# manyeyes/K2TransducerAsr

Measured on AMD Instinct MI355X. Metric: RTFx (audio-sec/wall-sec) offline Zipformer greedy, higher is better.
Workload: dtype f32

## Files before the change

### k2transducerasr_amd/csrc/attn.hip

```cpp
#include "kernels.h"

namespace k2hip {

typedef float f32x16 __attribute__((ext_vector_type(16)));

namespace {

constexpr int PH = 4;
constexpr int R = 32;

template <int NG>
__global__ __launch_bounds__(512, 4) void k_attn_scores_softmax(const float* __restrict__ qkp, int ld,
                                                             const float* __restrict__ pp, float* __restrict__ aw, int B,
                                                             int T, int Tp, int H, int lds_stride, int koff0, int poff0) {
    constexpr int QH = 8 * NG;
    extern __shared__ __attribute__((aligned(16))) float S[];
    const int tid = threadIdx.x, lane = tid & 63, wave = tid >> 6;
    const int li = lane & 31, lh = lane >> 5;
    const int i0 = blockIdx.x * R, b = blockIdx.y, h = blockIdx.z;
    const float* base = qkp + (long long)b * T * ld;
    const int qoff = h * QH, koff = koff0 + h * QH, poff = poff0 + h * PH;
    const int ppld = H * PH;

    float4 fq[NG];
// ... 111 lines not shown
                if (k >= nk) break;
                v[rr][k].x = __expf(v[rr][k].x - mx); v[rr][k].y = __expf(v[rr][k].y - mx);
                v[rr][k].z = __expf(v[rr][k].z - mx); v[rr][k].w = __expf(v[rr][k].w - mx);
                sum += (v[rr][k].x + v[rr][k].y) + (v[rr][k].z + v[rr][k].w);
            }
#pragma unroll
            for (int o = 32; o > 0; o >>= 1) sum += __shfl_xor(sum, o);
            const float inv = 1.0f / sum;
            float* orow = out + (long long)i * Tp;
#pragma unroll
            for (int k = 0; k < 4; k++) {
                const int j4 = lane * 4 + 256 * k;
                if (k < nk && j4 < Tp) *reinterpret_cast<float4*>(orow + j4) = make_float4(v[rr][k].x * inv, v[rr][k].y * inv, v[rr][k].z * inv, v[rr][k].w * inv);
            }
        }
        return;
    }
    for (int rr = 0; rr < 4; rr++) {
        int rl = wave * 4 + rr, i = i0 + rl;
        if (i >= T) break;
        float* srow = S + rl * lds_stride;
        float mx = -INFINITY;
        for (int j = lane; j < T; j += 64) mx = fmaxf(mx, srow[j]);
        mx = wave_max_dpp(mx);
        float sum = 0.f;
        for (int j = lane; j < T; j += 64) {
            float e = __expf(srow[j] - mx);
            srow[j] = e;
            sum += e;
        }
#pragma unroll
        for (int o = 32; o > 0; o >>= 1) sum += __shfl_xor(sum, o);
        float inv = 1.0f / sum;
        float* orow = out + (long long)i * Tp;
        for (int j4 = lane * 4; j4 < Tp; j4 += 256) {
            float4 v;
            v.x = (j4 + 0 < T) ? srow[j4 + 0] * inv : 0.f;
            v.y = (j4 + 1 < T) ? srow[j4 + 1] * inv : 0.f;
            v.z = (j4 + 2 < T) ? srow[j4 + 2] * inv : 0.f;
            v.w = (j4 + 3 < T) ? srow[j4 + 3] * inv : 0.f;
            *reinterpret_cast<float4*>(orow + j4) = v;
        }
    }
}

template <int NG>
__global__ __launch_bounds__(256) void k_attn_scores_softmax_long(const float* __restrict__ qkp, int ld, const float* __restrict__ pp,
                                                                  float* __restrict__ aw, int B, int T, int Tp, int H, int koff0, int poff0) {
    constexpr int QH = 8 * NG;
    __shared__ float smx[4][R], ssm[4][R];
    const int tid = threadIdx.x, lane = tid & 63, wave = tid >> 6;
    const int li = lane & 31, lh = lane >> 5;
    const int i0 = blockIdx.x * R, b = blockIdx.y, h = blockIdx.z;
    const float* base = qkp + (long long)b * T * ld;
    const int qoff = h * QH, koff = koff0 + h * QH, poff = poff0 + h * PH;
    const int ppld = H * PH;
    float4 fq[NG];
    {
        int row = i0 + li;
#pragma unroll
        for (int g = 0; g < NG; g++) {
            fq[g] = make_float4(0.f, 0.f, 0.f, 0.f);
            if (row < T) fq[g] = *reinterpret_cast<const float4*>(base + (long long)row * ld + qoff + 8 * g + 4 * lh);
        }
    }
    float4 pr[16];
#pragma unroll
    for (int r = 0; r < 16; r++) {
        int row = i0 + (r & 3) + 8 * (r >> 2) + 4 * lh;
        pr[r] = make_float4(0.f, 0.f, 0.f, 0.f);
        if (row < T) pr[r] = *reinterpret_cast<const float4*>(base + (long long)row * ld + poff);
    }
    const int njt = (T + 31) / 32;
    float rm[16], rs[16];
#pragma unroll
    for (int r = 0; r < 16; r++) { rm[r] = -INFINITY; rs[r] = 0.f; }
    float* out = aw + (((long long)h * B + b) * T) * Tp;
    for (int pass = 0; pass < 2; pass++) {
        for (int jt = wave; jt < njt; jt += 4) {
            const int j = jt * 32 + li;
            float4 fk[NG];
#pragma unroll
            for (int g = 0; g < NG; g++) {
                fk[g] = make_float4(0.f, 0.f, 0.f, 0.f);
                if (j < T) fk[g] = *reinterpret_cast<const float4*>(base + (long long)j * ld + koff + 8 * g + 4 * lh);
            }
            f32x16 acc;
#pragma unroll
            for (int r = 0; r < 16; r++) acc[r] = 0.f;
#pragma unroll
            for (int g = 0; g < NG; g++) {
                acc = __builtin_amdgcn_mfma_f32_32x32x2f32(fq[g].x, fk[g].x, acc, 0, 0, 0);
                acc = __builtin_amdgcn_mfma_f32_32x32x2f32(fq[g].y, fk[g].y, acc, 0, 0, 0);
                acc = __builtin_amdgcn_mfma_f32_32x32x2f32(fq[g].z, fk[g].z, acc, 0, 0, 0);
                acc = __builtin_amdgcn_mfma_f32_32x32x2f32(fq[g].w, fk[g].w, acc, 0, 0, 0);
            }
            if (j < T) {
#pragma unroll
                for (int r = 0; r < 16; r++) {
                    const int i = i0 + (r & 3) + 8 * (r >> 2) + 4 * lh;
                    if (i >= T) continue;
                    const float4 e = *reinterpret_cast<const float4*>(pp + (long long)(T - 1 - i + j) * ppld + h * PH);
                    const float sc = acc[r] + pr[r].x * e.x + pr[r].y * e.y + pr[r].z * e.z + pr[r].w * e.w;
                    if (pass == 0) {
                        const float m = fmaxf(rm[r], sc);
                        rs[r] = rs[r] * __expf(rm[r] - m) + __expf(sc - m);
                        rm[r] = m;
                    } else {
                        out[(long long)i * Tp + j] = __expf(sc - rm[r]) * rs[r];
                    }
                }
            }
        }
        if (pass == 0) {
#pragma unroll
            for (int r = 0; r < 16; r++) {
                float m = rm[r], sv = rs[r];
#pragma unroll
                for (int o = 16; o > 0; o >>= 1) {
                    const float om = __shfl_xor(m, o), os = __shfl_xor(sv, o);
                    const float nm = fmaxf(m, om);
                    sv = (m == -INFINITY ? 0.f : sv * __expf(m - nm)) + (om == -INFINITY ? 0.f : os * __expf(om - nm));
                    m = nm;
                }
                if (li == 0) {
                    const int rl = (r & 3) + 8 * (r >> 2) + 4 * lh;
                    smx[wave][rl] = m;
                    ssm[wave][rl] = sv;
                }
            }
            __syncthreads();
#pragma unroll
            for (int r = 0; r < 16; r++) {
                const int rl = (r & 3) + 8 * (r >> 2) + 4 * lh;
                float m = -INFINITY;
                for (int w = 0; w < 4; w++) m = fmaxf(m, smx[w][rl]);
                float sv = 0.f;
                for (int w = 0; w < 4; w++)
                    if (smx[w][rl] != -INFINITY) sv += ssm[w][rl] * __expf(smx[w][rl] - m);
                rm[r] = m;
                rs[r] = 1.0f / sv;
            }
        }
    }
    for (int idx = tid; idx < R * (Tp - T); idx += 256) {
        const int rl = idx / (Tp - T), c = T + idx % (Tp - T);
        if (i0 + rl < T) out[(long long)(i0 + rl) * Tp + c] = 0.f;
    }
}


typedef float f32x4 __attribute__((ext_vector_type(4)));

template <bool RING, bool PROJ = false>
__global__ __launch_bounds__(256) void k_attn_av_out(const float* __restrict__ aw, const float* __restrict__ v,
                                                     const float* __restrict__ wout, const float* __restrict__ bias,
                                                     float* __restrict__ x, int B, int T, int KL, int Tp, int Tk, int H, int vh,
                                                     int D, int tiles_per_z, RingRef ring, const float* __restrict__ newrows,
                                                     const float* __restrict__ xin = nullptr, const float* __restrict__ win = nullptr,
                                                     const float* __restrict__ bin = nullptr) {
    extern __shared__ float avs[];
    const int HV = H * vh, AS = HV + 1;
    const int tid = threadIdx.x, lane = tid & 63, wave = tid >> 6;
    const int b = blockIdx.y, i0 = blockIdx.x * 16;
    const int n = lane & 15, kq = lane >> 4;
    const float* xres = PROJ ? xin : x;
    if (RING) {
        float* rb = ring.pool + (long long)ring.slots[b] * ring.slot_stride + ring.off;
        const int head = (int)(((long long)ring.chunks[b] * T) % KL), h4 = HV >> 2;
        if (PROJ) {
            float* xs = avs + 16 * AS + ((4 - ((16 * AS) & 3)) & 3);
            const int XS = D + 4, d4 = D >> 2;
            for (int e = tid; e < 16 * d4; e += 256) {
                const int r = e / d4, c = (e % d4) * 4;
                *reinterpret_cast<float4*>(xs + r * XS + c) =
                    r < T ? *reinterpret_cast<const float4*>(xin + ((long long)b * T + r) * D + c) : make_float4(0.f, 0.f, 0.f, 0.f);
            }
            __syncthreads();
            const float* xr = xs + n * XS + 4 * kq;
            for (int ct = wave; 16 * ct < HV; ct += 4) {
                const int col = 16 * ct + n;
                const float* wr = win + (long long)min(col, HV - 1) * D + 4 * kq;
                f32x4 acc0 = {0.f, 0.f, 0.f, 0.f}, acc1 = {0.f, 0.f, 0.f, 0.f};
                for (int k0 = 0; k0 < D; k0 += 64) {
                    float4 w4[4], a4[4];
                    const int ns = min(4, (D - k0) >> 4);
#pragma unroll
                    for (int q = 0; q < 4; q++) w4[q] = q < ns ? *reinterpret_cast<const float4*>(wr + k0 + 16 * q) : make_float4(0.f, 0.f, 0.f, 0.f);
#pragma unroll
                    for (int q = 0; q < 4; q++) a4[q] = q < ns ? *reinterpret_cast<const float4*>(xr + k0 + 16 * q) : make_float4(0.f, 0.f, 0.f, 0.f);
#pragma unroll
                    for (int q = 0; q < 4; q += 2) {
                        acc0 = __builtin_amdgcn_mfma_f32_16x16x4f32(a4[q].x, w4[q].x, acc0, 0, 0, 0);
                        acc1 = __builtin_amdgcn_mfma_f32_16x16x4f32(a4[q + 1].x, w4[q + 1].x, acc1, 0, 0, 0);
                        acc0 = __builtin_amdgcn_mfma_f32_16x16x4f32(a4[q].y, w4[q].y, acc0, 0, 0, 0);
                        acc1 = __builtin_amdgcn_mfma_f32_16x16x4f32(a4[q + 1].y, w4[q + 1].y, acc1, 0, 0, 0);
                        acc0 = __builtin_amdgcn_mfma_f32_16x16x4f32(a4[q].z, w4[q].z, acc0, 0, 0, 0);
                        acc1 = __builtin_amdgcn_mfma_f32_16x16x4f32(a4[q + 1].z, w4[q + 1].z, acc1, 0, 0, 0);
                        acc0 = __builtin_amdgcn_mfma_f32_16x16x4f32(a4[q].w, w4[q].w, acc0, 0, 0, 0);
                        acc1 = __builtin_amdgcn_mfma_f32_16x16x4f32(a4[q + 1].w, w4[q + 1].w, acc1, 0, 0, 0);
                    }
                }
                if (col < HV) {
                    const float bc = bin[col];
#pragma unroll
                    for (int e = 0; e < 4; e++) {
                        const int r = 4 * kq + e;
                        if (r < T) rb[(long long)((head + r) % KL) * HV + col] = (acc0[e] + acc1[e]) + bc;
                    }
                }
            }
        } else {
            for (int e = tid; e < T * h4; e += 256) {
                const int r = e / h4, c = (e % h4) * 4;
                *reinterpret_cast<float4*>(rb + (long long)((head + r) % KL) * HV + c) =
                    *reinterpret_cast<const float4*>(newrows + ((long long)b * T + r) * HV + c);
            }
        }
        __syncthreads();
        v = rb;
    } else {
        v += (long long)b * KL * HV;
    }
    const int row_a = min(i0 + n, T - 1);
    const bool ncol = n < vh;
    for (int h = wave; h < H; h += 4) {
        const float* arow = aw + (((long long)h * B + b) * T + row_a) * Tp + 4 * kq;
        const float* vb = v + (long long)(4 * kq) * HV + h * vh + (ncol ? n : 0);
        f32x4 acc0 = {0.f, 0.f, 0.f, 0.f}, acc1 = {0.f, 0.f, 0.f, 0.f};
        float4 a4[4], a4n[4];
        float bv[4][4], bvn[4][4];
        auto load_step = [&](float4* ad, float (*bd)[4], int k0) {
#pragma unroll
            for (int g = 0; g < 4; g++) {
                const int kb = k0 + 16 * g + 4 * kq;
                ad[g] = kb < Tp ? *reinterpret_cast<const float4*>(arow + k0 + 16 * g) : make_float4(0.f, 0.f, 0.f, 0.f);
#pragma unroll
                for (int m = 0; m < 4; m++) bd[g][m] = (ncol && kb + m < KL) ? vb[(long long)(k0 + 16 * g + m) * HV] : 0.f;
            }
        };
        load_step(a4, bv, 0);
        for (int k0 = 0; k0 < Tk; k0 += 64) {
            if (k0 + 64 < Tk) load_step(a4n, bvn, k0 + 64);
#pragma unroll
            for (int g = 0; g < 4; g++) {
                if (g & 1) {
                    acc1 = __builtin_amdgcn_mfma_f32_16x16x4f32(a4[g].x, bv[g][0], acc1, 0, 0, 0);
                    acc1 = __builtin_amdgcn_mfma_f32_16x16x4f32(a4[g].y, bv[g][1], acc1, 0, 0, 0);
                    acc1 = __builtin_amdgcn_mfma_f32_16x16x4f32(a4[g].z, bv[g][2], acc1, 0, 0, 0);
                    acc1 = __builtin_amdgcn_mfma_f32_16x16x4f32(a4[g].w, bv[g][3], acc1, 0, 0, 0);
                } else {
                    acc0 = __builtin_amdgcn_mfma_f32_16x16x4f32(a4[g].x, bv[g][0], acc0, 0, 0, 0);
                    acc0 = __builtin_amdgcn_mfma_f32_16x16x4f32(a4[g].y, bv[g][1], acc0, 0, 0, 0);
                    acc0 = __builtin_amdgcn_mfma_f32_16x16x4f32(a4[g].z, bv[g][2], acc0, 0, 0, 0);
                    acc0 = __builtin_amdgcn_mfma_f32_16x16x4f32(a4[g].w, bv[g][3], acc0, 0, 0, 0);
                }
            }
#pragma unroll
            for (int g = 0; g < 4; g++) {
                a4[g] = a4n[g];
#pragma unroll
                for (int m = 0; m < 4; m++) bv[g][m] = bvn[g][m];
            }
        }
        if (ncol) {
#pragma unroll
            for (int e = 0; e < 4; e++) avs[(4 * kq + e) * AS + h * vh + n] = acc0[e] + acc1[e];
        }
    }
    __syncthreads();
    constexpr int MAXC = 8;
    const int nch = (HV + 15) >> 4;
    float4 av4[MAXC];
#pragma unroll
    for (int c = 0; c < MAXC; c++) {
        const int kb = 16 * c + 4 * kq;
        const float* ar = avs + n * AS + kb;
        av4[c] = (c < nch && kb < HV) ? make_float4(ar[0], ar[1], ar[2], ar[3]) : make_float4(0.f, 0.f, 0.f, 0.f);
    }
    const int ct0 = blockIdx.z * tiles_per_z, ct1 = min(D >> 4, ct0 + tiles_per_z);
    float4 wc[MAXC], wn[MAXC];
    auto load_w = [&](float4* dst, int ct) {
        const float* wr = wout + (long long)(ct * 16 + n) * HV + 4 * kq;
#pragma unroll
        for (int c = 0; c < MAXC; c++)
            dst[c] = (c < nch && 16 * c + 4 * kq < HV) ? *reinterpret_cast<const float4*>(wr + 16 * c) : make_float4(0.f, 0.f, 0.f, 0.f);
    };
    float xa[4], xb[4], ba = 0.f, bb = 0.f;
    auto load_x = [&](float* dst, float& bdst, int ct) {
        const int col = ct * 16 + n;
        bdst = bias[col];
#pragma unroll
        for (int e = 0; e < 4; e++) {
            const int i = i0 + 4 * kq + e;
            dst[e] = i < T ? xres[((long long)b * T + i) * D + col] : 0.f;
        }
    };
    auto tile = [&](const float4* w, const float* xr, float bv, int ct) {
        const int col = ct * 16 + n;
        f32x4 acc0 = {0.f, 0.f, 0.f, 0.f}, acc1 = {0.f, 0.f, 0.f, 0.f};
#pragma unroll
        for (int c = 0; c < MAXC; c++) {
            if (c < nch) {
                if (c & 1) {
                    acc1 = __builtin_amdgcn_mfma_f32_16x16x4f32(av4[c].x, w[c].x, acc1, 0, 0, 0);
                    acc1 = __builtin_amdgcn_mfma_f32_16x16x4f32(av4[c].y, w[c].y, acc1, 0, 0, 0);
                    acc1 = __builtin_amdgcn_mfma_f32_16x16x4f32(av4[c].z, w[c].z, acc1, 0, 0, 0);
                    acc1 = __builtin_amdgcn_mfma_f32_16x16x4f32(av4[c].w, w[c].w, acc1, 0, 0, 0);
                } else {
                    acc0 = __builtin_amdgcn_mfma_f32_16x16x4f32(av4[c].x, w[c].x, acc0, 0, 0, 0);
                    acc0 = __builtin_amdgcn_mfma_f32_16x16x4f32(av4[c].y, w[c].y, acc0, 0, 0, 0);
                    acc0 = __builtin_amdgcn_mfma_f32_16x16x4f32(av4[c].z, w[c].z, acc0, 0, 0, 0);
                    acc0 = __builtin_amdgcn_mfma_f32_16x16x4f32(av4[c].w, w[c].w, acc0, 0, 0, 0);
                }
            }
        }
        float o[4];
#pragma unroll
        for (int e = 0; e < 4; e++) o[e] = acc0[e] + acc1[e] + bv + xr[e];
        asm volatile("" : "+v"(o[0]), "+v"(o[1]), "+v"(o[2]), "+v"(o[3]));
        float* xp = x + ((long long)b * T + i0 + 4 * kq) * D + col;
#pragma unroll
        for (int e = 0; e < 4; e++)
            if (i0 + 4 * kq + e < T) xp[(long long)e * D] = o[e];
    };
    int ct = ct0 + wave;
    if (ct < ct1) {
        load_w(wc, ct);
        load_x(xa, ba, ct);
    }
    while (ct < ct1) {
        if (ct + 4 < ct1) {
            load_w(wn, ct + 4);
            load_x(xb, bb, ct + 4);
        }
        tile(wc, xa, ba, ct);
        ct += 4;
        if (ct >= ct1) break;
        if (ct + 4 < ct1) {
            load_w(wc, ct + 4);
            load_x(xa, ba, ct + 4);
        }
        tile(wn, xb, bb, ct);
        ct += 4;
    }
}


template <int NS, int NT, bool MULTI = false>
__global__ __launch_bounds__(NT) void k_nonlin_av_out(const float* __restrict__ aw, const float* __restrict__ hid, int ldh,
                                                      const float* __restrict__ wout, const float* __restrict__ bias,
                                                      float* __restrict__ x, int B, int T, int KL, int Tp, int Hc, int D,
                                                      int tiles_per_z, RingRef ring) {
    extern __shared__ float cs_[];
    constexpr int NWV = NT / 64;
    const int CS = ((Hc + 15) & ~15) + 4;
    const int tid = threadIdx.x, lane = tid & 63, wave = tid >> 6;
    const int b = blockIdx.y;
    const int n = lane & 15, kq = lane >> 4;
    float* rb = ring.pool + (long long)ring.slots[b] * ring.slot_stride + ring.off;
    {
        const int head = (int)(((long long)ring.chunks[b] * T) % KL), h4 = Hc >> 2;
        for (int e = tid; e < T * h4; e += NT) {
            const int r = e / h4, c = (e % h4) * 4;
            const float* p = hid + ((long long)b * T + r) * ldh + c;
            const float4 sg = *reinterpret_cast<const float4*>(p), v = *reinterpret_cast<const float4*>(p + Hc);
            *reinterpret_cast<float4*>(rb + (long long)((head + r) % KL) * Hc + c) =
                make_float4(v.x * tanhf(sg.x), v.y * tanhf(sg.y), v.z * tanhf(sg.z), v.w * tanhf(sg.w));
        }
    }
    __syncthreads();
    const int row_a = min(n, T - 1);
    const float* arow = aw + ((long long)b * T + row_a) * Tp + 4 * kq;
    for (int ct = wave; ct * 16 < Hc; ct += NWV) {
        const bool cok = ct * 16 + n < Hc;
        const float* vb = rb + (long long)(4 * kq) * Hc + (cok ? ct * 16 + n : 0);
        f32x4 acc0 = {0.f, 0.f, 0.f, 0.f}, acc1 = {0.f, 0.f, 0.f, 0.f};
        const int trips = MULTI ? (KL + 64 * NS - 1) / (64 * NS) : 1;
        for (int tr = 0; tr < trips; tr++) {
        const int k0 = 64 * NS * tr;
        float4 a4[NS][4];
        float bv[NS][4][4];
#pragma unroll
        for (int s = 0; s < NS; s++)
#pragma unroll
            for (int g = 0; g < 4; g++) {
                const int kb = k0 + 64 * s + 16 * g + 4 * kq;
                a4[s][g] = kb < Tp ? *reinterpret_cast<const float4*>(arow + k0 + 64 * s + 16 * g) : make_float4(0.f, 0.f, 0.f, 0.f);
#pragma unroll
                for (int m = 0; m < 4; m++) bv[s][g][m] = (cok && kb + m < KL) ? vb[(long long)(k0 + 64 * s + 16 * g + m) * Hc] : 0.f;
            }
#pragma unroll
        for (int s = 0; s < NS; s++)
#pragma unroll
            for (int g = 0; g < 4; g++) {
                if (g & 1) {
                    acc1 = __builtin_amdgcn_mfma_f32_16x16x4f32(a4[s][g].x, bv[s][g][0], acc1, 0, 0, 0);
                    acc1 = __builtin_amdgcn_mfma_f32_16x16x4f32(a4[s][g].y, bv[s][g][1], acc1, 0, 0, 0);
                    acc1 = __builtin_amdgcn_mfma_f32_16x16x4f32(a4[s][g].z, bv[s][g][2], acc1, 0, 0, 0);
                    acc1 = __builtin_amdgcn_mfma_f32_16x16x4f32(a4[s][g].w, bv[s][g][3], acc1, 0, 0, 0);
                } else {
                    acc0 = __builtin_amdgcn_mfma_f32_16x16x4f32(a4[s][g].x, bv[s][g][0], acc0, 0, 0, 0);
                    acc0 = __builtin_amdgcn_mfma_f32_16x16x4f32(a4[s][g].y, bv[s][g][1], acc0, 0, 0, 0);
                    acc0 = __builtin_amdgcn_mfma_f32_16x16x4f32(a4[s][g].z, bv[s][g][2], acc0, 0, 0, 0);
                    acc0 = __builtin_amdgcn_mfma_f32_16x16x4f32(a4[s][g].w, bv[s][g][3], acc0, 0, 0, 0);
                }
            }
        }
#pragma unroll
        for (int e = 0; e < 4; e++) {
            const int r = 4 * kq + e;
            const float gate = (cok && r < T) ? hid[((long long)b * T + r) * ldh + 2 * Hc + ct * 16 + n] : 0.f;
            cs_[r * CS + ct * 16 + n] = (acc0[e] + acc1[e]) * gate;
        }
    }
    __syncthreads();
    if (!wout) {
        const int h4 = Hc >> 2;
        for (int e = tid; e < T * h4; e += NT) {
            const int r = e / h4, c = (e % h4) * 4;
            *reinterpret_cast<float4*>(x + ((long long)b * T + r) * Hc + c) = *reinterpret_cast<const float4*>(cs_ + r * CS + c);
        }
        return;
    }
    const int ct0 = blockIdx.z * tiles_per_z, ct1 = min(D >> 4, ct0 + tiles_per_z);
    const float* ar = cs_ + n * CS + 4 * kq;
    for (int ct = ct0 + wave; ct < ct1; ct += NWV) {
        const int col = ct * 16 + n;
        const float* wr = wout + (long long)col * Hc + 4 * kq;
        const float bvv = bias[col];
        float xr[4];
#pragma unroll
        for (int e = 0; e < 4; e++) {
            const int i = 4 * kq + e;
            xr[e] = i < T ? x[((long long)b * T + i) * D + col] : 0.f;
        }
        f32x4 acc0 = {0.f, 0.f, 0.f, 0.f}, acc1 = {0.f, 0.f, 0.f, 0.f};
        for (int c0 = 0; c0 < Hc; c0 += 64) {
            float4 w4[4], a4[4];
#pragma unroll
            for (int g = 0; g < 4; g++) {
                const bool ok = c0 + 16 * g + 4 * kq < Hc;
                w4[g] = ok ? *reinterpret_cast<const float4*>(wr + c0 + 16 * g) : make_float4(0.f, 0.f, 0.f, 0.f);
                a4[g] = ok ? *reinterpret_cast<const float4*>(ar + c0 + 16 * g) : make_float4(0.f, 0.f, 0.f, 0.f);
            }
#pragma unroll
            for (int g = 0; g < 4; g++) {
                if (g & 1) {
                    acc1 = __builtin_amdgcn_mfma_f32_16x16x4f32(a4[g].x, w4[g].x, acc1, 0, 0, 0);
                    acc1 = __builtin_amdgcn_mfma_f32_16x16x4f32(a4[g].y, w4[g].y, acc1, 0, 0, 0);
                    acc1 = __builtin_amdgcn_mfma_f32_16x16x4f32(a4[g].z, w4[g].z, acc1, 0, 0, 0);
                    acc1 = __builtin_amdgcn_mfma_f32_16x16x4f32(a4[g].w, w4[g].w, acc1, 0, 0, 0);
                } else {
                    acc0 = __builtin_amdgcn_mfma_f32_16x16x4f32(a4[g].x, w4[g].x, acc0, 0, 0, 0);
                    acc0 = __builtin_amdgcn_mfma_f32_16x16x4f32(a4[g].y, w4[g].y, acc0, 0, 0, 0);
                    acc0 = __builtin_amdgcn_mfma_f32_16x16x4f32(a4[g].z, w4[g].z, acc0, 0, 0, 0);
                    acc0 = __builtin_amdgcn_mfma_f32_16x16x4f32(a4[g].w, w4[g].w, acc0, 0, 0, 0);
                }
            }
        }
        float o[4];
#pragma unroll
        for (int e = 0; e < 4; e++) o[e] = acc0[e] + acc1[e] + bvv + xr[e];
        float* xp = x + ((long long)b * T + 4 * kq) * D + col;
#pragma unroll
        for (int e = 0; e < 4; e++)
            if (4 * kq + e < T) xp[(long long)e * D] = o[e];
    }
}

}

template <int NG>
static void attn_scores_launch(const Ctx& ctx, const float* qkp, int ld, const float* pp, float* aw, int B, int T, int Tp, int H, int koff0,
                               int poff0) {
    int lds_stride = Tp + 4;
    size_t lds = sizeof(float) * R * lds_stride;
    const bool force_long = tunables().attn_long != 0;
    if (lds > 160 * 1024 || force_long) {
        hipLaunchKernelGGL(k_attn_scores_softmax_long<NG>, dim3(cdiv(T, R), B, H), dim3(256), 0, ctx.stream, qkp, ld, pp, aw, B, T, Tp, H, koff0,
                           poff0);
        K2_HIP(hipGetLastError());
        return;
    }
    static LdsAttrOnce lds_attr;
    lds_attr.ensure(k_attn_scores_softmax<NG>, 160 * 1024);
    dim3 grid(cdiv(T, R), B, H);
    hipLaunchKernelGGL(k_attn_scores_softmax<NG>, grid, dim3(512), lds, ctx.stream, qkp, ld, pp, aw, B, T, Tp, H, lds_stride, koff0, poff0);
    K2_HIP(hipGetLastError());
}

void attn_scores_softmax(const Ctx& ctx, const float* qkp, int ld, const float* pp, float* aw, int B, int T, int Tp, int H, int qh, int koff0,
                         int poff0) {
    K2_REQUIRE(Tp % 4 == 0 && Tp >= T, "attn: Tp=%d must be T=%d rounded up to 4", Tp, T);
    if (koff0 < 0) koff0 = H * qh;
    if (poff0 < 0) poff0 = 2 * H * qh;
    K2_REQUIRE(koff0 % 4 == 0 && poff0 % 4 == 0 && ld % 4 == 0, "attn: operand offsets must be multiples of 4 floats");
    ctx.add_flops(0.0, 2.0 * (qh + PH) * (double)T * T * B * H, 0);
    if (ctx.dry) return;
    switch (qh) {
        case 32: attn_scores_launch<4>(ctx, qkp, ld, pp, aw, B, T, Tp, H, koff0, poff0); break;
        case 24: attn_scores_launch<3>(ctx, qkp, ld, pp, aw, B, T, Tp, H, koff0, poff0); break;
        case 16: attn_scores_launch<2>(ctx, qkp, ld, pp, aw, B, T, Tp, H, koff0, poff0); break;
        default: failf(K2HIP_ERR_UNSUPPORTED, "attention head size %d unsupported (16, 24, 32)", qh);
    }
}

bool attn_av_out(const Ctx& ctx, const float* aw, const float* v, const float* wout, const float* bias, float* x, int B, int T, int KL, int Tp,
                 int H, int vh, int D) {
    const int HV = H * vh, Tk = (KL + 63) & ~63;
    const bool off = tunables().no_fused_av != 0;
    if (off || vh > 16 || HV % 4 != 0 || HV > 128 || D % 16 != 0 || Tp % 4 != 0 || Tp < KL) return false;
    ctx.add_flops(0.0, 2.0 * B * (double)T * HV * (KL + D), 0);
    if (ctx.dry) return true;
    const int strips = cdiv(T, 16) * B, ntile = D / 16;
    int cs = std::max(1, std::min(4, 512 / std::max(1, strips)));
    cs = std::min(cs, ntile);
    const int tiles_per_z = cdiv(ntile, cs);
    cs = cdiv(ntile, tiles_per_z);
    const size_t lds = sizeof(float) * 16 * (HV + 1);
    hipLaunchKernelGGL(k_attn_av_out<false>, dim3(cdiv(T, 16), B, cs), dim3(256), lds, ctx.stream, aw, v, wout, bias, x, B, T, KL, Tp, Tk, H, vh,
                       D, tiles_per_z, RingRef(), nullptr);
    K2_HIP(hipGetLastError());
    return true;
}

bool attn_av_out_ring(const Ctx& ctx, const float* aw, const RingRef& vals, const float* newrows, const float* wout, const float* bias, float* x,
                      int B, int T, int KL, int Tp, int H, int vh, int D) {
    const int HV = H * vh, Tk = (KL + 63) & ~63;
    K2_REQUIRE(vh <= 16 && HV % 4 == 0 && HV <= 128 && D % 16 == 0 && Tp % 4 == 0 && Tp >= KL && T <= 16,
               "attn_av_out_ring: shape H=%d vh=%d D=%d T=%d KL=%d unsupported", H, vh, D, T, KL);
    ctx.add_flops(0.0, 2.0 * B * (double)T * HV * (KL + D), 0);
    if (ctx.dry) return true;
    const int strips = B, ntile = D / 16;
    int cs = std::max(1, std::min(4, 512 / std::max(1, strips)));
    cs = std::min(cs, ntile);
    const int tiles_per_z = cdiv(ntile, cs);
    cs = cdiv(ntile, tiles_per_z);
    const size_t lds = sizeof(float) * 16 * (HV + 1);
    hipLaunchKernelGGL(k_attn_av_out<true>, dim3(1, B, cs), dim3(256), lds, ctx.stream, aw, nullptr, wout, bias, x, B, T, KL, Tp, Tk, H, vh, D,
                       tiles_per_z, vals, newrows);
    K2_HIP(hipGetLastError());
    return true;
}

void attn_proj_av_out_ring(const Ctx& ctx, const float* aw, const RingRef& vals, const float* xin, const float* win, const float* bin,
                           const float* wout, const float* bias, float* xout, int B, int T, int KL, int Tp, int H, int vh, int D) {
    const int HV = H * vh, Tk = (KL + 63) & ~63;
    K2_REQUIRE(vh <= 16 && HV % 4 == 0 && HV <= 128 && D % 32 == 0 && Tp % 4 == 0 && Tp >= KL && T <= 16,
               "attn_proj_av_out_ring: shape H=%d vh=%d D=%d T=%d KL=%d unsupported", H, vh, D, T, KL);
    K2_REQUIRE(ctx.dry || xin != xout, "attn_proj_av_out_ring: input and output must be different buffers");
    ctx.add_flops(0.0, 2.0 * B * (double)T * HV * (KL + D) + 2.0 * B * (double)T * HV * D, 0);
    if (ctx.dry) return;
    const int strips = B, ntile = D / 16;
    int cs = std::max(1, std::min(4, 512 / std::max(1, strips)));
    cs = std::min(cs, ntile);
    const int tiles_per_z = cdiv(ntile, cs);
    cs = cdiv(ntile, tiles_per_z);
    const size_t lds = sizeof(float) * (16 * (HV + 1) + 4 + 16 * (D + 4));
    K2_REQUIRE(lds <= 64 * 1024, "attn_proj_av_out_ring: D=%d too wide", D);
    hipLaunchKernelGGL((k_attn_av_out<true, true>), dim3(1, B, cs), dim3(256), lds, ctx.stream, aw, nullptr, wout, bias, xout, B, T, KL, Tp, Tk, H, vh,
                       D, tiles_per_z, vals, nullptr, xin, win, bin);
    K2_HIP(hipGetLastError());
}

void nonlin_av_out_ring(const Ctx& ctx, const float* aw, const RingRef& cache, const float* hid, int ldh, const float* wout, const float* bias,
                        float* x, int B, int T, int KL, int Tp, int Hc, int D) {
    K2_REQUIRE(Hc % 4 == 0 && D % 16 == 0 && Tp % 4 == 0 && Tp >= KL && T <= 16 && ldh % 4 == 0 && ldh >= 3 * Hc,
               "nonlin_av_out_ring: shape Hc=%d D=%d T=%d KL=%d unsupported", Hc, D, T, KL);
    ctx.add_flops(0.0, 2.0 * B * (double)T * Hc * (KL + D), 0);
    const size_t lds = sizeof(float) * 16 * (((Hc + 15) & ~15) + 4);
    K2_REQUIRE(lds <= 64 * 1024, "nonlin_av_out_ring: Hc=%d too wide", Hc);
    const int ns = (KL + 63) / 64;
    K2_REQUIRE(ns >= 1, "nonlin_av_out_ring: no keys");
    if (ctx.dry) return;
    const int ntile = D / 16;
    int cs = std::max(1, std::min(4, 512 / std::max(1, B)));
    cs = std::min(cs, ntile);
    if (!wout) cs = 1;
    const int tiles_per_z = cdiv(ntile, cs);
    cs = cdiv(ntile, tiles_per_z);
    const bool wide = (Hc + 15) / 16 > 8;
#define K2_NONLIN_LAUNCH(NS_, NT_)                                                                                                   \
    hipLaunchKernelGGL((k_nonlin_av_out<NS_, NT_>), dim3(1, B, cs), dim3(NT_), lds, ctx.stream, aw, hid, ldh, wout, bias, x, B, T, KL, Tp, Hc, \
                       D, tiles_per_z, cache)
    switch (ns) {
        case 1: if (wide) K2_NONLIN_LAUNCH(1, 1024); else K2_NONLIN_LAUNCH(1, 512); break;
        case 2: if (wide) K2_NONLIN_LAUNCH(2, 1024); else K2_NONLIN_LAUNCH(2, 512); break;
        case 3: if (wide) K2_NONLIN_LAUNCH(3, 1024); else K2_NONLIN_LAUNCH(3, 512); break;
        case 4: K2_NONLIN_LAUNCH(4, 512); break;
        default:
            hipLaunchKernelGGL((k_nonlin_av_out<4, 512, true>), dim3(1, B, cs), dim3(512), lds, ctx.stream, aw, hid, ldh, wout, bias, x, B, T, KL,
                               Tp, Hc, D, tiles_per_z, cache);
            break;
    }
#undef K2_NONLIN_LAUNCH
    K2_HIP(hipGetLastError());
}

}
```

### k2transducerasr_amd/csrc/kernels.h

```cpp
#pragma once
#include "ctc_prefix_layout.h"
#include "common.h"

namespace k2hip {

#ifdef K2HIP_DEV
#define K2HIP_DEV_SWITCH(name, def) int name = def
#else
#define K2HIP_DEV_SWITCH(name, def) static constexpr int name = def
#endif
struct Tunables {
    int no_glu_epilogue = 0;
    int attn_long = 0;
    int no_fused_av = 0;
    int fused_vproj_min_t = 4;
    int no_fused_vproj = 0;
    int no_fused_conv = 0;
    int conformer_gemm_scores = 0;
    int dw7_tiled = 0;
    int dw1d_tt = 0;
    int lstm_seq = 0;
    int greedy_one_part = 0;
    int greedy_parts = 0;
    int beam_launches = 0;
    int beam_parts = 0;
    int beam_hyp_global = 0;
    int beam_trace = 0;
    int search_rounds = -1;
    int test_greedy_timeout = 0;
    int decoder_table_mb = 1024;
    int screen_min_v = 1024;
    int screen_count = 0;
    int max_streams = 0;
    K2HIP_DEV_SWITCH(gemm_cfg, -1);
    K2HIP_DEV_SWITCH(xcd_panels, 0);
    K2HIP_DEV_SWITCH(greedy_stamps, 0);
    K2HIP_DEV_SWITCH(conformer_stamps, 0);
};
void tunables_init_from_env();
const Tunables& tunables();
bool tunables_set(const char* env_name, int value);

struct GemmStats {
    double flops = 0;
    double total_flops = 0;
    int launches = 0;
    float ms = 0;
};

struct GemmLaunchRec {
    int M, N, K, batch, act, res, kind;
    float us;
};

struct GreedyLaunch;
struct Ctx {
    std::vector<GemmLaunchRec>* gemm_log = nullptr;
    GreedyLaunch* greedy_rec = nullptr;
    hipStream_t stream = nullptr;
    Arena* arena = nullptr;
    bool dry = false;
    bool one_part = false;
    bool instrument = false;
    GemmStats* stats = nullptr;
    std::vector<hipEvent_t>* evpool = nullptr;
    int* evused = nullptr;
    hipEvent_t next_event() const {
        if ((size_t)*evused == evpool->size()) {
            hipEvent_t e;
            K2_HIP(hipEventCreate(&e));
            evpool->push_back(e);
        }
        return (*evpool)[(*evused)++];
    }
    void add_flops(double gemm_fl, double other_fl, int launches) const {
        if (stats && dry) {
            stats->flops += gemm_fl;
            stats->total_flops += gemm_fl + other_fl;
            stats->launches += launches;
        }
    }
};

enum Act : int { ACT_NONE = 0, ACT_SWOOSH_L = 1, ACT_SWOOSH_R = 2, ACT_TANH = 3, ACT_SIGMOID = 4, ACT_RELU = 5, ACT_DOUBLE_SWISH = 6 };

struct GemmArgs {
    const float* A = nullptr;
    const float* W = nullptr;
    const float* bias = nullptr;
    const float* res = nullptr;
    float* C = nullptr;
    int M = 0, N = 0, K = 0;
    int lda = 0, ldw = 0, ldc = 0, ldr = 0;
    int act = ACT_NONE;
    int xcd_panels = 0;
    int act_cols = 0;
    int w_kn = 0;
    int nb0 = 1, nb1 = 1;
    const int* skip_if_zero = nullptr;
    long long sA0 = 0, sA1 = 0, sW0 = 0, sW1 = 0, sC0 = 0, sC1 = 0, sR0 = 0, sR1 = 0;
    long long sBias0 = 0;
    int cv_Fout = 0, cv_Tout = 0, cv_Tin = 0, cv_Fin = 0, cv_C = 0, cv_st = 1, cv_sf = 1;
    int seg_len = 0, seg_stride = 0;
    int res_div = 1;
    int act_after_res = 0;
    int glu = 0;
    int glu_cols = 0;
    const float* mul = nullptr;
    int ldm = 0;
    long long sM0 = 0, sM1 = 0;
    const float* byp_orig = nullptr;
    const float* byp_scale = nullptr;
    int ld_orig = 0;
    float* cf_pool = nullptr;
    long long cf_stride = 0, cf_off = 0;
    const int* cf_slots = nullptr;
    const float *cf_wc = nullptr, *cf_bc = nullptr, *cf_ww = nullptr, *cf_bw = nullptr, *cf_sc = nullptr;
    int cf_Tc = 0, cf_K = 0;
    unsigned long long* dbg = nullptr;
    int ablate = 0;
};
void gemm(const Ctx& ctx, const GemmArgs& a);
bool gemm_glu_causal_conv(const Ctx& ctx, const float* x, const float* wg, const float* bg, float* pool, long long slot_stride, long long off,
                          const int* slots, const float* wc, const float* bc, const float* ww, const float* bw, const float* sc, float* y, int B,
                          int Tc, int D, int K);

#define K2_PIPE_TABLE(X)                                                                                                       \
    X(0, 128, 64, 64, 32, 3) X(1, 128, 64, 32, 32, 3) X(2, 128, 128, 64, 64, 3) X(3, 128, 128, 64, 32, 3) X(4, 128, 64, 64, 32, 4)  \
    X(5, 64, 64, 32, 32, 3) X(6, 128, 128, 64, 64, 4) X(7, 64, 128, 32, 64, 3) X(8, 128, 128, 32, 32, 3) X(9, 128, 64, 32, 32, 4) \
    X(10, 64, 64, 64, 32, 3) X(11, 64, 64, 32, 64, 3) X(12, 256, 64, 64, 32, 3) X(13, 128, 32, 32, 32, 3) X(14, 128, 32, 64, 32, 3)
#define K2_P16_TABLE(X) X(0, 64, 96, 32, 48, 3) X(1, 128, 96, 64, 48, 3) X(2, 64, 192, 32, 96, 3) X(3, 32, 96, 16, 48, 3)
#define K2_RING_TABLE(X)                                                                                        \
    X(0, 128, 64, 1, 2, 0, 0) X(1, 128, 64, 1, 3, 0, 0) X(2, 128, 64, 1, 2, 0, 1) X(3, 128, 64, 1, 3, 0, 1) X(4, 128, 64, 1, 4, 0, 1)   \
    X(5, 64, 64, 1, 3, 0, 0) X(6, 64, 64, 1, 3, 0, 1) X(7, 64, 64, 1, 4, 0, 1) X(8, 64, 64, 2, 3, 0, 0) X(9, 64, 64, 2, 3, 0, 1)      \
    X(10, 64, 64, 4, 2, 0, 0) X(11, 64, 64, 4, 2, 0, 1) X(12, 32, 64, 2, 3, 0, 0) X(13, 32, 64, 4, 3, 0, 0) X(14, 32, 64, 4, 3, 0, 1)  \
    X(15, 32, 32, 4, 3, 0, 0) X(16, 32, 32, 4, 4, 0, 1) X(17, 64, 32, 4, 3, 0, 0) X(18, 128, 128, 1, 2, 0, 0) X(19, 128, 128, 1, 2, 0, 1) \
    X(20, 64, 128, 1, 3, 0, 0) X(21, 64, 128, 1, 3, 0, 1) X(22, 64, 96, 1, 3, 0, 0) X(23, 64, 96, 1, 3, 0, 1) X(24, 128, 96, 1, 2, 0, 1) \
    X(25, 128, 64, 1, 3, 2, 0) X(26, 128, 64, 1, 3, 2, 1) X(27, 128, 64, 2, 2, 0, 1) X(28, 64, 96, 2, 3, 0, 0) X(29, 64, 96, 2, 2, 0, 0) \
    X(30, 64, 96, 2, 2, 0, 1) X(31, 128, 96, 1, 3, 0, 0) X(32, 128, 96, 1, 3, 0, 1)
struct RingCfg { int BM, BN, KS, NST, LW, PF; };
#define X(i, bm, bn, ks, nst, lw, pf) {bm, bn, ks, nst, lw, pf},
constexpr RingCfg kRing[] = {K2_RING_TABLE(X)};
#undef X
#define K2_DMA_TABLE(X)                                                                                                          \
    X(0, 128, 128, 64, 32, 3) X(5, 128, 64, 32, 32, 2) X(8, 128, 64, 32, 32, 4) X(9, 64, 64, 32, 32, 2) X(10, 64, 64, 32, 32, 3) \
    X(11, 64, 96, 32, 32, 2) X(20, 32, 32, 32, 32, 4) X(21, 32, 64, 32, 32, 4)
#define K2_REG_TABLE(X)                                                                                                           \
    X(0, 128, 128, 64, 32, 32) X(1, 128, 128, 64, 32, 64) X(2, 64, 64, 32, 32, 32) X(3, 64, 64, 32, 32, 64) X(4, 128, 64, 32, 32, 64) \
    X(5, 128, 64, 32, 32, 32) X(12, 128, 32, 32, 32, 32)
enum GemmMode { MODE_PLAIN = 0, MODE_CONV = 1, MODE_WKN = 2 };

enum class GemmFamily { REG, DMA, PIPE, P16, RING, SKINNY3, SKINNY6, SKINNY6_8 };
struct GemmPlan {
    GemmFamily family = GemmFamily::REG;
    int idx = 0;
    int mode = MODE_PLAIN;
    int ablate = 0;
    int BM = 0, BN = 0, waves = 0;
};
struct GemmForce {
    enum Kind { AUTO, CFG, RING, PIPE, P16 } kind = AUTO;
    int idx = -1;
    int ablate = 0;
    bool dma = true;
};
GemmForce decode_gemm_force(int code);
GemmPlan plan_gemm(const GemmArgs& a, const GemmForce& f);
int gemm_kind(const GemmArgs& a, const GemmPlan& p);
// ... 450 lines not shown
```

### k2transducerasr_amd/csrc/tunables.cpp

```cpp
#include <cstdlib>
#include <cstring>
#include <mutex>

#include "kernels.h"

namespace k2hip {

namespace {
constexpr int kMaxDev = 64;
std::mutex g_util_mu[kMaxDev];
hipStream_t g_util_stream[kMaxDev] = {};
hipError_t util_device(int* dev) {
    hipError_t e = hipGetDevice(dev);
    if (e != hipSuccess) return e;
    return (*dev < 0 || *dev >= kMaxDev) ? hipErrorInvalidDevice : hipSuccess;
}
hipError_t util_stream(int dev, hipStream_t* s) {
    if (!g_util_stream[dev]) {
        hipError_t e = hipStreamCreateWithFlags(&g_util_stream[dev], hipStreamNonBlocking);
        if (e != hipSuccess) return e;
    }
    *s = g_util_stream[dev];
    return hipSuccess;
}
}
hipError_t copy_blocking(void* dst, const void* src, size_t bytes, hipMemcpyKind kind) {
    if (bytes == 0) return hipSuccess;
    int dev = 0;
    hipError_t e = util_device(&dev);
    if (e != hipSuccess) return e;
    std::lock_guard<std::mutex> lk(g_util_mu[dev]);
    hipStream_t s = nullptr;
    e = util_stream(dev, &s);
    if (e != hipSuccess) return e;
    e = hipMemcpyAsync(dst, src, bytes, kind, s);
    if (e != hipSuccess) return e;
    return hipStreamSynchronize(s);
}
hipError_t fill_blocking(void* dst, int value, size_t bytes) {
    if (bytes == 0) return hipSuccess;
    int dev = 0;
    hipError_t e = util_device(&dev);
    if (e != hipSuccess) return e;
    std::lock_guard<std::mutex> lk(g_util_mu[dev]);
    hipStream_t s = nullptr;
    e = util_stream(dev, &s);
    if (e != hipSuccess) return e;
    e = hipMemsetAsync(dst, value, bytes, s);
    if (e != hipSuccess) return e;
    return hipStreamSynchronize(s);
}

namespace {
Tunables g_t;
bool g_init = false;
struct Entry {
    const char* env;
    int Tunables::*field;
    bool flag;
};
const Entry kEntries[] = {
    {"K2HIP_NO_GLU_EPILOGUE", &Tunables::no_glu_epilogue, true},
    {"K2HIP_ATTN_LONG", &Tunables::attn_long, true},
    {"K2HIP_NO_FUSED_AV", &Tunables::no_fused_av, true},
    {"K2HIP_NO_FUSED_VPROJ", &Tunables::no_fused_vproj, true},
    {"K2HIP_FUSED_VPROJ_MIN_T", &Tunables::fused_vproj_min_t, false},
    {"K2HIP_NO_FUSED_CONV", &Tunables::no_fused_conv, true},
    {"K2HIP_CONFORMER_GEMM_SCORES", &Tunables::conformer_gemm_scores, true},
    {"K2HIP_DW7_TILED", &Tunables::dw7_tiled, true},
    {"K2HIP_DW1D_TT", &Tunables::dw1d_tt, false},
    {"K2HIP_LSTM_SEQ", &Tunables::lstm_seq, true},
    {"K2HIP_GREEDY_ONE_PART", &Tunables::greedy_one_part, true},
    {"K2HIP_GREEDY_PARTS", &Tunables::greedy_parts, false},
    {"K2HIP_DECODER_TABLE_MB", &Tunables::decoder_table_mb, false},
    {"K2HIP_BEAM_LAUNCHES", &Tunables::beam_launches, true},
    {"K2HIP_BEAM_HYP_GLOBAL", &Tunables::beam_hyp_global, true},
    {"K2HIP_BEAM_PARTS", &Tunables::beam_parts, false},
    {"K2HIP_BEAM_TRACE", &Tunables::beam_trace, true},
    {"K2HIP_SCREEN_MIN_V", &Tunables::screen_min_v, false},
    {"K2HIP_SCREEN_COUNT", &Tunables::screen_count, false},
    {"K2HIP_TEST_GREEDY_TIMEOUT", &Tunables::test_greedy_timeout, true},
    {"K2HIP_SEARCH_ROUNDS", &Tunables::search_rounds, false},
    {"K2HIP_MAX_STREAMS", &Tunables::max_streams, false},
#ifdef K2HIP_DEV
    {"K2HIP_GEMM_CFG", &Tunables::gemm_cfg, false},
    {"K2HIP_XCD_PANELS", &Tunables::xcd_panels, false},
    {"K2HIP_GREEDY_STAMPS", &Tunables::greedy_stamps, true},
    {"K2HIP_CONFORMER_STAMPS", &Tunables::conformer_stamps, true},
#endif
};
}

void tunables_init_from_env() {
    static std::once_flag once;
    std::call_once(once, [] {
    g_init = true;
    for (const Entry& e : kEntries)
        if (const char* v = getenv(e.env)) g_t.*(e.field) = e.flag ? 1 : atoi(v);
    });
}

const Tunables& tunables() { return g_t; }
bool tunables_set(const char* env_name, int value) {
    for (const Entry& e : kEntries)
        if (!strcmp(e.env, env_name)) {
            g_t.*(e.field) = value;
            return true;
        }
    return false;
}

}
```

Before: 23940.

## Stage V tiles in LDS with double buffering for the fused attention AV kernel

```diff
diff --git a/k2transducerasr_amd/csrc/attn.hip b/k2transducerasr_amd/csrc/attn.hip
--- a/k2transducerasr_amd/csrc/attn.hip
+++ b/k2transducerasr_amd/csrc/attn.hip
@@ -287,7 +287,7 @@
 
 typedef float f32x4 __attribute__((ext_vector_type(4)));
 
-template <bool RING, bool PROJ = false>
+template <bool RING, bool PROJ = false, int VLDS = 0>
 __global__ __launch_bounds__(256) void k_attn_av_out(const float* __restrict__ aw, const float* __restrict__ v,
                                                      const float* __restrict__ wout, const float* __restrict__ bias,
                                                      float* __restrict__ x, int B, int T, int KL, int Tp, int Tk, int H, int vh,
@@ -359,6 +359,97 @@
     }
     const int row_a = min(i0 + n, T - 1);
     const bool ncol = n < vh;
+    if (VLDS) {
+        constexpr int NI = VLDS == 3 ? 3 : 4;
+        const int VP = ((min(H, 4) * vh + 15) & ~15) + 4;
+        float* vs = avs + ((16 * AS + 3) & ~3);
+        const int sr = tid >> 2, sq = 4 * (tid & 3);
+        for (int r = tid; r < 128; r += 256) vs[r * VP + VP - 1] = 0.f;
+        for (int h0 = 0; h0 < H; h0 += 4) {
+            const int c0 = h0 * vh, CW = min(4, H - h0) * vh;
+            const int h = min(h0 + wave, H - 1);
+            const float* arow = aw + (((long long)h * B + b) * T + row_a) * Tp;
+            const float* vg = v + c0;
+            const float* lb = vs + (4 * kq) * VP + (ncol && h0 + wave < H ? wave * vh + n : VP - 1);
+            int sc[NI];
+#pragma unroll
+            for (int i = 0; i < NI; i++) sc[i] = min(sq + 16 * i, CW - 4);
+            f32x4 acc0 = {0.f, 0.f, 0.f, 0.f}, acc1 = {0.f, 0.f, 0.f, 0.f};
+            float4 a4[4], a4n[4], s4[NI];
+            auto load_v = [&](int k0) {
+                const float* vr = vg + (long long)min(k0 + sr, KL - 1) * HV;
+#pragma unroll
+                for (int i = 0; i < NI; i++) s4[i] = *reinterpret_cast<const float4*>(vr + sc[i]);
+            };
+            auto store_v = [&](float* dst, int k0) {
+                const bool in = k0 + sr < KL;
+#pragma unroll
+                for (int i = 0; i < NI; i++) {
+                    float4 t = s4[i];
+                    asm volatile("" : "+v"(t.x), "+v"(t.y), "+v"(t.z), "+v"(t.w));
+                    *reinterpret_cast<float4*>(dst + sr * VP + sc[i]) = in ? t : make_float4(0.f, 0.f, 0.f, 0.f);
+                }
+            };
+            auto load_a = [&](float4* ad, int k0) {
+#pragma unroll
+                for (int g = 0; g < 4; g++) ad[g] = *reinterpret_cast<const float4*>(arow + min(k0 + 16 * g + 4 * kq, Tp - 4));
+            };
+            auto zero_a = [&](float4* ad, int k0) {
+#pragma unroll
+                for (int g = 0; g < 4; g++) {
+                    asm volatile("" : "+v"(ad[g].x), "+v"(ad[g].y), "+v"(ad[g].z), "+v"(ad[g].w));
+                    if (k0 + 16 * g + 4 * kq >= Tp) ad[g] = make_float4(0.f, 0.f, 0.f, 0.f);
+                }
+            };
+            auto step = [&](const float* lc) {
+                float bb[4][4];
+#pragma unroll
+                for (int g = 0; g < 4; g++)
+#pragma unroll
+                    for (int m = 0; m < 4; m++) bb[g][m] = lc[(16 * g + m) * VP];
+                __builtin_amdgcn_sched_barrier(0);
+#pragma unroll
+                for (int g = 0; g < 4; g++) {
+                    const float b0 = bb[g][0], b1 = bb[g][1], b2 = bb[g][2], b3 = bb[g][3];
+                    if (g & 1) {
+                        acc1 = __builtin_amdgcn_mfma_f32_16x16x4f32(a4[g].x, b0, acc1, 0, 0, 0);
+                        acc1 = __builtin_amdgcn_mfma_f32_16x16x4f32(a4[g].y, b1, acc1, 0, 0, 0);
+                        acc1 = __builtin_amdgcn_mfma_f32_16x16x4f32(a4[g].z, b2, acc1, 0, 0, 0);
+                        acc1 = __builtin_amdgcn_mfma_f32_16x16x4f32(a4[g].w, b3, acc1, 0, 0, 0);
+                    } else {
+                        acc0 = __builtin_amdgcn_mfma_f32_16x16x4f32(a4[g].x, b0, acc0, 0, 0, 0);
+                        acc0 = __builtin_amdgcn_mfma_f32_16x16x4f32(a4[g].y, b1, acc0, 0, 0, 0);
+                        acc0 = __builtin_amdgcn_mfma_f32_16x16x4f32(a4[g].z, b2, acc0, 0, 0, 0);
+                        acc0 = __builtin_amdgcn_mfma_f32_16x16x4f32(a4[g].w, b3, acc0, 0, 0, 0);
+                    }
+                }
+            };
+            load_v(0);
+            load_a(a4, 0);
+            store_v(vs, 0);
+            zero_a(a4, 0);
+            __syncthreads();
+            int cur = 0;
+            for (int k0 = 0; k0 + 64 < Tk; k0 += 64, cur ^= 1) {
+                load_v(k0 + 64);
+                load_a(a4n, k0 + 64);
+                __builtin_amdgcn_sched_barrier(0);
+                step(lb + cur * 64 * VP);
+                __builtin_amdgcn_sched_barrier(0);
+                store_v(vs + (cur ^ 1) * 64 * VP, k0 + 64);
+                zero_a(a4n, k0 + 64);
+#pragma unroll
+                for (int g = 0; g < 4; g++) a4[g] = a4n[g];
+                __syncthreads();
+            }
+            step(lb + cur * 64 * VP);
+            if (ncol && h0 + wave < H) {
+#pragma unroll
+                for (int e = 0; e < 4; e++) avs[(4 * kq + e) * AS + h * vh + n] = acc0[e] + acc1[e];
+            }
+            __syncthreads();
+        }
+    } else
     for (int h = wave; h < H; h += 4) {
         const float* arow = aw + (((long long)h * B + b) * T + row_a) * Tp + 4 * kq;
         const float* vb = v + (long long)(4 * kq) * HV + h * vh + (ncol ? n : 0);
@@ -404,7 +495,7 @@
         }
     }
     __syncthreads();
-    constexpr int MAXC = 8;
+    constexpr int MAXC = VLDS == 3 ? 4 : 8;
     const int nch = (HV + 15) >> 4;
     float4 av4[MAXC];
 #pragma unroll
@@ -654,8 +745,19 @@
     const int tiles_per_z = cdiv(ntile, cs);
     cs = cdiv(ntile, tiles_per_z);
     const size_t lds = sizeof(float) * 16 * (HV + 1);
-    hipLaunchKernelGGL(k_attn_av_out<false>, dim3(cdiv(T, 16), B, cs), dim3(256), lds, ctx.stream, aw, v, wout, bias, x, B, T, KL, Tp, Tk, H, vh,
-                       D, tiles_per_z, RingRef(), nullptr);
+    if (KL >= tunables().av_lds_min_t) {
+        const int VP = ((std::min(H, 4) * vh + 15) & ~15) + 4;
+        const size_t lds_long = sizeof(float) * (((16 * (HV + 1) + 3) & ~3) + 2 * 64 * VP);
+        if (HV <= 48)
+            hipLaunchKernelGGL((k_attn_av_out<false, false, 3>), dim3(cdiv(T, 16), B, cs), dim3(256), lds_long, ctx.stream, aw, v, wout, bias, x, B,
+                               T, KL, Tp, Tk, H, vh, D, tiles_per_z, RingRef(), nullptr);
+        else
+            hipLaunchKernelGGL((k_attn_av_out<false, false, 4>), dim3(cdiv(T, 16), B, cs), dim3(256), lds_long, ctx.stream, aw, v, wout, bias, x, B,
+                               T, KL, Tp, Tk, H, vh, D, tiles_per_z, RingRef(), nullptr);
+    } else {
+        hipLaunchKernelGGL(k_attn_av_out<false>, dim3(cdiv(T, 16), B, cs), dim3(256), lds, ctx.stream, aw, v, wout, bias, x, B, T, KL, Tp, Tk, H,
+                           vh, D, tiles_per_z, RingRef(), nullptr);
+    }
     K2_HIP(hipGetLastError());
     return true;
 }
diff --git a/k2transducerasr_amd/csrc/kernels.h b/k2transducerasr_amd/csrc/kernels.h
--- a/k2transducerasr_amd/csrc/kernels.h
+++ b/k2transducerasr_amd/csrc/kernels.h
@@ -14,6 +14,7 @@
     int attn_long = 0;
     int no_fused_av = 0;
     int fused_vproj_min_t = 4;
+    int av_lds_min_t = 64;
     int no_fused_vproj = 0;
     int no_fused_conv = 0;
     int conformer_gemm_scores = 0;
diff --git a/k2transducerasr_amd/csrc/tunables.cpp b/k2transducerasr_amd/csrc/tunables.cpp
--- a/k2transducerasr_amd/csrc/tunables.cpp
+++ b/k2transducerasr_amd/csrc/tunables.cpp
@@ -65,6 +65,7 @@
     {"K2HIP_NO_FUSED_AV", &Tunables::no_fused_av, true},
     {"K2HIP_NO_FUSED_VPROJ", &Tunables::no_fused_vproj, true},
     {"K2HIP_FUSED_VPROJ_MIN_T", &Tunables::fused_vproj_min_t, false},
+    {"K2HIP_AV_LDS_MIN_T", &Tunables::av_lds_min_t, false},
     {"K2HIP_NO_FUSED_CONV", &Tunables::no_fused_conv, true},
     {"K2HIP_CONFORMER_GEMM_SCORES", &Tunables::conformer_gemm_scores, true},
     {"K2HIP_DW7_TILED", &Tunables::dw7_tiled, true},
```

Result: no change. 24090, median of 6 (+0.6%).
